# MarioPasc/MGA-YOLO

Hardware: AMD Instinct MI355X
Metric: images/s (MaskCBAM fwd+bwd step at P3/P4/P5, YOLOv8n 640x640) (higher is better)
Workload: dtype f32; 1 GPU; YOLOv8n+MGA-CBAM P3/P4/P5, 32x640x640 synthetic per GPU, fp32 (BASELINE.json configs[1]); batch_per_gpu=32, global_batch=32, parallelism=dp1, launch=hipGraph replay, 1 graph/step, handoff_kernels=True

## Files before the change

mga_yolo_amd/csrc/api_bwd.hip:

```cpp
#include "host.cuh"
#include "bwd.cuh"
#include "nhwc_bwd.cuh"

static int backward_args(const mgacbam_bwd_level_t& L, NhwcBwdArgs& N, Sig& sig) {
  const bool nhwc = (L.flags & MGACBAM_LAYOUT_NHWC) != 0;
  if (!L.x || !L.gy || !L.ctx || !L.scratch || !L.gx) return fail(MGACBAM_E_NULL, "backward: x / gy / ctx / scratch / gx is NULL");
  if (!L.gw1 || !L.gb1 || !L.gw2 || !L.gb2 || !L.gwsa || !L.gbeta) return fail(MGACBAM_E_NULL, "backward: NULL parameter-gradient pointer");
  if (L.gmask && !L.mask) return fail(MGACBAM_E_NULL, "backward: gmask requested but mask is NULL");
  if (int e = check_level("backward", L)) return e;
  const int VEC = level_vec(nhwc, L.C, L.H, L.W, L.dtype);
  const size_t need = VEC * elem_size(L.dtype);
  if (!aligned_to(L.x, need) || !aligned_to(L.gy, need) || !aligned_to(L.gx, need) || !aligned_to(L.ctx, 16) ||
      !aligned_to(L.scratch, 16) || (L.gmask && !aligned_to(L.gmask, nhwc ? 4 : 16)) || (nhwc && L.mask && !aligned_to(L.mask, 4)))
    return fail(MGACBAM_E_ALIGN, "backward%s: x/gy/gx must be %zu-byte aligned, ctx/scratch 16-byte", nhwc ? " (NHWC)" : "", need);
  const ScratchLayout SL = scratch_layout(L.B, L.C, L.H, L.W, L.p.hidden, L.p.k, nhwc, VEC);
  if (int e = check_ctx_capacity("backward", L)) return e;
  if (int e = check_capacity("backward", "scratch", SL.total, L.scratch_bytes)) return e;
  BwdArgs& A = N.a;
  A.x = L.x; A.mask = L.mask; A.gy = L.gy; A.gx = L.gx; A.gmask = L.gmask;
  A.gw1 = L.gw1; A.gb1 = L.gb1; A.gw2 = L.gw2; A.gb2 = L.gb2; A.gwsa = L.gwsa; A.gbeta = L.gbeta;
  level_setup(L, A);
  A.s = scratch_ptrs(L.scratch, SL);
  A.nconv = A.g.B * conv_tiles(A.t, A.g.H, A.g.W);
  A.nwsa = A.g.B * wsa_tiles(A.t, A.g.H, A.g.W);
  A.npg = params_blocks(A.g);
  A.merged = 0;
  A.make_proj = 0;
  A.vec = VEC;
  sig = Sig{L.dtype, VEC, L.mask != nullptr, L.p.k, L.gmask != nullptr, 0};
  if (nhwc) {
    N.n = nhwc_geo(L.C, L.H, L.W, VEC);
    N.ncb = (L.C + kNhwcFoldC - 1) / kNhwcFoldC;
    A.nt = N.n.nchunk;
    A.ncg = N.ncb;
    A.bflag0 = A.cflag0 = A.mbflag0 = A.mcflag0 = A.wflag0 = A.sflag0 = 0;
    sig.nhwc = 1;
    sig.weight = L.C;
    return 0;
  }
  A.nt = chan_tiles(A.t, A.g.H, A.g.W, VEC);
  A.ncg = 0;
  const SyncLayout S = sync_layout(L.B, L.C, static_cast<size_t>(L.H) * L.W);
  A.bflag0 = static_cast<int>(S.bflag); A.cflag0 = static_cast<int>(S.cflag);
  A.mbflag0 = static_cast<int>(S.mbflag); A.mcflag0 = static_cast<int>(S.mcflag);
  A.wflag0 = static_cast<int>(S.wflag); A.sflag0 = static_cast<int>(S.sflag);
  sig.weight = L.C * A.t.chan_tx;
  const bool have = (L.flags & MGACBAM_BWD_HAVE_PROJ) != 0;
  const bool make = !have && L.dtype == MGACBAM_F32 && reduce1_smem(A.g, VEC, true) <= 64 * 1024;
  sig.proj = L.gmask != nullptr;
  A.g.proj_h = (L.gmask && L.p.hidden <= MGACBAM_PROJ_MAX_HIDDEN && (have || make)) ? L.p.hidden : 0;
  A.make_proj = A.g.proj_h > 0 && make;
  return 0;
}

static size_t reduce2_smem(const Tune& t) { return (64 + static_cast<size_t>(std::max(kPghLds, kBlock / t.pool_tx))) * sizeof(float); }
static int launch_convT(Group<BwdArgs>& G, int k, hipStream_t st) {
  auto kernel = with_k(k, [](auto kk) { return k_bwd_convT<kk.value>; });
  return launch_group("k_bwd_convT", kernel, G, [](const BwdArgs& a) { return a.nconv; }, [&](const BwdArgs& a) { return convT_smem(a.t, k); }, st);
}
static int launch_wsa(Group<BwdArgs>& G, int k, hipStream_t st) {
  auto kernel = with_k(k, [](auto kk) { return k_bwd_wsa<kk.value>; });
  return launch_group("k_bwd_wsa", kernel, G, [](const BwdArgs& a) { return a.nwsa; }, [&](const BwdArgs& a) { return wsa_smem(a.t, k); }, st);
}
static int launch_params(Group<BwdArgs>& G, hipStream_t st) {
  return launch_group("k_bwd_params", k_bwd_params, G, [](const BwdArgs& a) { return a.npg; }, [](const BwdArgs& a) { return params_smem(a.g); }, st);
}

static int backward_group(BwdArgs* lv, int n, const Sig& sig, int stages, hipStream_t st) {
  constexpr int kReduce2MaxCpt = 4;
  const int cpt = group_cpt(lv, n, kReduce2MaxCpt);
  for (int l = 0; l < n; ++l) {
    lv[l].t.pool_cpt = cpt;
    const int cpb = (kBlock / lv[l].t.pool_tx) * cpt;
    lv[l].ncg = (lv[l].g.C + cpb - 1) / cpb;
  }
  Group<BwdArgs> G = make_group(lv, n);

  bool fold = (stages & MGACBAM_BWD_FOLD) && (stages & MGACBAM_BWD_REDUCE1) && (stages & MGACBAM_BWD_CONVT);
  for (int l = 0; l < n && fold; ++l) {
    const int TP = lv[l].t.chan_tx * sig.vec;
    fold = TP >= kSyncPx && TP >= lv[l].g.W && 8 * (((lv[l].t.conv_th + lv[l].g.k) * lv[l].g.W + TP - 1) / TP + 1) <= 512 &&
           lv[l].nconv <= lv[l].g.B * lv[l].nflag;
  }
  bool mkproj = false;
// ... 23 lines not shown
      return with_bool(mkproj, [&](auto pj) { return k_bwd_r12<elem_t<decltype(t)>, v.value, c.value, pj.value>; }); }); });
    if (int e = launch("k_bwd_r12", kernel, tot, kBlock, smem, st, R)) return e;
    for (int l = 0; l < n; ++l) G.lv[l] = lv[l];
  }
  if (fold && !merge) {
    auto kernel = with_elem_vec(sig.dtype, sig.vec, [&](auto t, auto v) { return with_k7(sig.k, [&](auto k) {
      return with_bool(mkproj, [&](auto pj) { return k_bwd_reduce1_fold<elem_t<decltype(t)>, v.value, k.value, pj.value>; }); }); });
    if (int e = launch_group("k_bwd_reduce1_fold", kernel, G, [](const BwdArgs& a) { return xcd_grid(a.g.B, a.nt) + pad8(a.nconv); },
                             [&](const BwdArgs& a) { return std::max(reduce1_smem(a.g, sig.vec, a.make_proj), convT_smem(a.t, sig.k)); },
                             st)) return e;
  }
  if ((stages & MGACBAM_BWD_REDUCE1) && !fold) {
    auto kernel = with_elem_vec(sig.dtype, sig.vec, [&](auto t, auto v) {
      return with_bool(mkproj, [&](auto pj) { return k_bwd_reduce1<elem_t<decltype(t)>, v.value, pj.value>; }); });
    if (int e = launch_group("k_bwd_reduce1", kernel, G, [](const BwdArgs& a) { return xcd_grid(a.g.B, a.nt); },
                             [&](const BwdArgs& a) { return reduce1_smem(a.g, sig.vec, a.make_proj); }, st)) return e;
  }
  if ((stages & MGACBAM_BWD_CONVT) && !fold)
    if (int e = launch_convT(G, sig.k, st)) return e;
  const bool fuse_pg = fuse && (stages & MGACBAM_BWD_APPLY) && (stages & MGACBAM_BWD_PARAMGRAD);
  const bool fuse_wsa = fuse && (stages & MGACBAM_BWD_REDUCE2) && (stages & MGACBAM_BWD_WSA) && sig.k == 7;
  if ((stages & MGACBAM_BWD_REDUCE2) && !merge) {
    auto kernel = with_elem_vec(sig.dtype, sig.vec, [&](auto t, auto v) { return with_cpt(cpt, [&](auto c) {
      return with_bool(fuse_wsa, [&](auto fw) { return k_bwd_reduce2<elem_t<decltype(t)>, v.value, c.value, fw.value>; }); }); });
    if (int e = launch_group("k_bwd_reduce2", kernel, G,
                             [&](const BwdArgs& a) { return (fuse_wsa ? pad8(a.nwsa) : 0) + sweep_blocks(a, a.t.pool_tx, cpt); },
                             [&](const BwdArgs& a) { return std::max(reduce2_smem(a.t), fuse_wsa ? wsa_smem(a.t, sig.k) : 0); }, st)) return e;
  }
  if ((stages & MGACBAM_BWD_WSA) && !fuse_wsa && !merge)
    if (int e = launch_wsa(G, sig.k, st)) return e;
  if ((stages & MGACBAM_BWD_PARAMGRAD) && !fuse_pg)
    if (int e = launch_params(G, st)) return e;
  if (stages & MGACBAM_BWD_APPLY) {
    auto kernel = with_elem_vec(sig.dtype, sig.vec, [&](auto t, auto v) { return with_bool(sig.gmask, [&](auto gm) {
      return with_bool(fuse_pg, [&](auto pg) { return k_bwd_apply<elem_t<decltype(t)>, v.value, gm.value, pg.value>; }); }); });
    if (int e = launch_group("k_bwd_apply", kernel, G, [&](const BwdArgs& a) { return (fuse_pg ? pad8(a.npg) : 0) + xcd_grid(a.g.B, a.nt); },
                             [&](const BwdArgs& a) { return std::max(bwd_apply_smem(a.g, sig.vec), fuse_pg ? params_smem(a.g) : 0); }, st)) return e;
  }
  return 0;
}

static int backward_group_nhwc(NhwcBwdArgs* lv, int n, const Sig& sig, int stages, hipStream_t st) {
  Group<NhwcBwdArgs> G = make_group(lv, n);
  Group<BwdArgs> GB;
  GB.n = n;
  for (int l = 0; l < n; ++l) GB.lv[l] = lv[l].a;
  auto chunks = [](const NhwcBwdArgs& a) { return xcd_grid(a.a.g.B, a.n.nchunk); };
  if (stages & MGACBAM_BWD_REDUCE1) {
    auto kernel = with_elem_vec8(sig.dtype, sig.vec, [](auto t, auto v) { return k_bwd_reduce1_nhwc<elem_t<decltype(t)>, v.value>; });
    if (int e = launch_group("k_bwd_reduce1_nhwc", kernel, G, chunks,
                             [&](const NhwcBwdArgs& a) { return nhwc_reduce1_smem(a.a.g, sig.vec); }, st)) return e;
  }
  if (stages & MGACBAM_BWD_CONVT)
    if (int e = launch_convT(GB, sig.k, st)) return e;
  if (stages & MGACBAM_BWD_REDUCE2) {
    auto kernel = with_elem_vec8(sig.dtype, sig.vec, [](auto t, auto v) { return k_bwd_reduce2_nhwc<elem_t<decltype(t)>, v.value>; });
    if (int e = launch_group("k_bwd_reduce2_nhwc", kernel, G, chunks, [](const NhwcBwdArgs& a) { return nhwc_reduce2_smem(a.a.g); }, st)) return e;
    if (int e = launch_group("k_bwd_fold_nhwc", k_bwd_fold_nhwc, G, [](const NhwcBwdArgs& a) { return a.a.g.B * a.ncb; }, 0, st)) return e;
  }
  if (stages & MGACBAM_BWD_WSA)
    if (int e = launch_wsa(GB, sig.k, st)) return e;
  if (stages & MGACBAM_BWD_PARAMGRAD)
    if (int e = launch_params(GB, st)) return e;
  if (stages & MGACBAM_BWD_APPLY) {
    auto kernel = with_elem_vec8(sig.dtype, sig.vec, [&](auto t, auto v) {
      return with_bool(sig.gmask, [&](auto gm) { return k_bwd_apply_nhwc<elem_t<decltype(t)>, v.value, gm.value>; }); });
    if (int e = launch_group("k_bwd_apply_nhwc", kernel, G, [](const NhwcBwdArgs& a) { return xcd_grid(a.a.g.B, a.n.ntile); },
                             [](const NhwcBwdArgs& a) { return nhwc_bwd_apply_smem(a.a.g); }, st)) return e;
// ... 14 lines not shown
```

mga_yolo_amd/csrc/args.cuh:

```cuda
#pragma once
#include <stddef.h>
#include <stdint.h>

namespace mgacbam {

struct Geo {
  int B, C, H, W, HW;
  int hidden, k;
  int use_sigmoid;
  float thr, eps;
  int proj_h;
};
constexpr int kProjMax = 4;
constexpr int kGateR = 16;
constexpr int kSyncPx = 16;

struct CtxPtrs {
  float* S; float* use; float* den;
  float* avg; float* mx; float* mavg;
  int* valid; int* amax;
  float* h_avg; float* h_mx; float* ca;
  float* planes; int* cidx; float* sa;
  float* proj;
  int* sync;
};

struct ParamPtrs { const float* w1; const float* b1; const float* w2; const float* b2; const float* wsa; const float* beta; };

struct Tune {
  int pool_tx;
  int pool_cpt;
  int chan_tx;
  int conv_twq;
  int conv_th;
  int wsa_th;
  int apply_rows;
  int gate_rows;
  int gate_tx;
  int gate_span;
};

struct FwdArgs {
  const void* x; const float* mask; void* y;
  CtxPtrs c; ParamPtrs p; Geo g; Tune t;
  int nflag;
  int fused;
  unsigned spin_limit;
  int fault;
  long long* trace;
};

struct ScratchPtrs {
  float* A_part;
  float* gpre;
  float* gplanes;
  float* gwsa_part;
  float* gz;
  float* gbq;
  float* gh_avg;
  float* gh_mx;
  float* pgh;
};

struct BwdArgs {
  const void* x; const float* mask; const void* gy; void* gx; float* gmask;
  float* gw1; float* gb1; float* gw2; float* gb2; float* gwsa; float* gbeta;
  CtxPtrs c; ParamPtrs p; ScratchPtrs s; Geo g; Tune t;
  int nt;
  int nconv;
  int nwsa;
  int npg;
  int ncg;
  int nflag;
  int bflag0;
  int cflag0;
  int wflag0;
  int sflag0;
  int mbflag0, mcflag0;
  int make_proj;
  int merged;
  unsigned spin_limit;
  int vec;
  long long* trace;
};

struct NhwcGeo {
  int cs, lcs;
  int ng;
  int ch;
  int ntile;
  int rp;
  int nchunk;
};
constexpr int kNhwcMaxChunks = 64;
// ... 14 lines not shown
```

mga_yolo_amd/csrc/bwd.cuh:

```cuda
#pragma once
#include "args.cuh"
#include "common.cuh"
#include "tile.cuh"

namespace mgacbam {

constexpr int kPghLds = 2048;

template <typename T, int VEC, bool FOLD = false, bool PROJ = false>
__device__ __forceinline__ void bwd_reduce1_body(const BwdArgs& A, const int bid, float* smem) {
  constexpr int HP = kProjMax;
  static_assert(HP % 4 == 0, "the W1 rows of a channel are read as float4");
  const Geo& g = A.g;
  const int tid = threadIdx.x;
  const int TX = A.t.chan_tx, lt = ilog2(TX);
  const int tx = tid & (TX - 1), ty = tid >> lt, TY = kBlock >> lt;
  const int nv = g.HW / VEC;
  const int ntile = A.nt;
  int b, tile;
  if (!xcd_sample_part(bid, g.B, ntile, b, tile)) return;
  const int i = tile * TX + tx;
  const bool active = i < nv;
  const int ii = active ? i : nv - 1;
  const size_t base = static_cast<size_t>(b) * g.C * g.HW + static_cast<size_t>(ii) * VEC;
  const T* xp = static_cast<const T*>(A.x) + base;
  const T* gp = static_cast<const T*>(A.gy) + base;
  const float a = softplusf_(*A.p.beta);
  float* s_ca = smem;
  float* s_aq = smem + g.C;
  const bool proj = PROJ && A.make_proj;
  float* s_w1t = smem + ((3 * g.C + 3) & ~3);
  float* sm = proj ? s_w1t + g.C * HP : s_aq + 2 * g.C;
  for (int c = tid; c < g.C; c += kBlock) s_ca[c] = A.c.ca[static_cast<size_t>(b) * g.C + c];
  if (PROJ) {
    if (proj) {
      for (int idx = tid; idx < g.C * HP; idx += kBlock) {
        const int c = idx / HP, j = idx - c * HP;
        s_w1t[idx] = j < g.proj_h ? A.p.w1[static_cast<size_t>(j) * g.C + c] : 0.f;
      }
    }
  }

  float sav[VEC];
  load_vec<float, VEC>(A.c.sa + static_cast<size_t>(b) * g.HW + static_cast<size_t>(ii) * VEC, sav);
  const float live = active ? 1.f : 0.f;
  float accp[VEC];
#pragma unroll
  for (int e = 0; e < VEC; ++e) accp[e] = 0.f;
  float accP[PROJ ? HP : 1][VEC];
#pragma unroll
  for (int j = 0; j < (PROJ ? HP : 1); ++j)
#pragma unroll
    for (int e = 0; e < VEC; ++e) accP[j][e] = 0.f;
  __syncthreads();

#pragma unroll 4
  for (int c = ty; c < g.C; c += TY) {
    float xv[VEC], gv[VEC];
    load_vec<T, VEC>(xp + static_cast<size_t>(c) * g.HW, xv);
    load_vec<T, VEC>(gp + static_cast<size_t>(c) * g.HW, gv);
    const float cac = s_ca[c];
    if (PROJ) {
      if (proj) {
        float w[HP];
#pragma unroll
        for (int q4 = 0; q4 < HP / 4; ++q4) {
          const float4 wv = *reinterpret_cast<const float4*>(s_w1t + c * HP + 4 * q4);
          w[4 * q4] = wv.x; w[4 * q4 + 1] = wv.y; w[4 * q4 + 2] = wv.z; w[4 * q4 + 3] = wv.w;
        }
#pragma unroll
        for (int j = 0; j < HP; ++j)
#pragma unroll
          for (int e = 0; e < VEC; ++e) accP[j][e] += w[j] * xv[e];
      }
    }
    float pa = 0.f, pq = 0.f;
#pragma unroll
    for (int e = 0; e < VEC; ++e) {
      const float p = xv[e] * gv[e] * live;
      accp[e] += cac * p;
      pa += p * sav[e];
      pq += p * (cac * sav[e] - 1.f);
    }
    pa = wave_group_sum(pa, TX);
    pq = wave_group_sum(pq, TX);
    if (tx == 0) { s_aq[c] = pa; s_aq[g.C + c] = pq; }
  }
#pragma unroll
  for (int e = 0; e < VEC; ++e) sm[tid * VEC + e] = accp[e];
  __syncthreads();
// ... 16 lines not shown
    } else {
      store_vec<float, VEC>(gq, gpre);
    }
  }
  if (FOLD) handoff_publish(A.c.sync + A.bflag0 + static_cast<size_t>(b) * A.nflag + tile);
  if (PROJ) {
    if (proj) {
#pragma unroll
      for (int half = 0; half < HP / 4; ++half) {
        if (half * 4 >= g.proj_h) break;
        if (!FOLD || half) __syncthreads();
#pragma unroll
        for (int jj = 0; jj < 4; ++jj)
#pragma unroll
          for (int e = 0; e < VEC; ++e) sm[(jj * kBlock + tid) * VEC + e] = accP[half * 4 + jj][e];
        __syncthreads();
        if (ty == 0 && active) {
#pragma unroll
          for (int jj = 0; jj < 4; ++jj) {
            const int j = half * 4 + jj;
            if (j < g.proj_h) {
              float pv[VEC];
#pragma unroll
              for (int e = 0; e < VEC; ++e) pv[e] = accP[j][e];
              for (int r = 1; r < TY; ++r)
#pragma unroll
                for (int e = 0; e < VEC; ++e) pv[e] += sm[(jj * kBlock + r * TX + tx) * VEC + e];
              store_vec<float, VEC>(A.c.proj + (static_cast<size_t>(b) * g.proj_h + j) * g.HW + static_cast<size_t>(i) * VEC, pv);
            }
          }
        }
      }
    }
  }
}

template <typename T, int VEC, bool PROJ>
__global__ __launch_bounds__(kBlock) void k_bwd_reduce1(const Group<BwdArgs> G) {
  extern __shared__ __align__(16) float smem[];
  int local;
  const int l = find_level(G, blockIdx.x, local);
  bwd_reduce1_body<T, VEC, false, PROJ>(G.lv[l], local, smem);
}

template <int K, bool COH>
__device__ __forceinline__ void bwd_convT_body(const BwdArgs& A, const int local, float* smem) {
  const Geo& g = A.g;
  const int k = K ? K : g.k;
  const ConvTile c = conv_tile(g, A.t, k, local, A.t.conv_th);
  const int tid = threadIdx.x;
  float* wts = smem;
  float* tg = smem + ((3 * k * k + 3) & ~3);
  for (int i = tid; i < 3 * k * k; i += kBlock) wts[i] = A.p.wsa[i];
  const float* gpre = A.s.gpre + static_cast<size_t>(c.b) * g.HW;
  bool bad = false;
  if (COH) {
    int* own = A.c.sync + A.cflag0 + local;
    const int gen = static_cast<int>(static_cast<unsigned>(ld_agent(own)) + 1u);
    const int TP = A.t.chan_tx * A.vec;
    const int ra = max(c.y0 - c.pad, 0), rb = min(c.y0 + c.TH - 1 + c.pad, g.H - 1);
    bad = handoff_wait(A.c.sync + A.bflag0 + static_cast<size_t>(c.b) * A.nflag, (ra * g.W) / TP, ((rb + 1) * g.W - 1) / TP, gen,
                       A.c.sync + static_cast<size_t>(g.B) * A.nflag, A.spin_limit);
    if (tid == 0 && !A.merged) __hip_atomic_fetch_add(own, 1, __ATOMIC_RELAXED, __HIP_MEMORY_SCOPE_AGENT);
  }
  stage_window<8>(tg, 1, c.PH, c.PW, c.y0 - c.pad, c.x0 - c.pad, g, [&](int, int off) { return COH ? ld_agent(gpre + off) : gpre[off]; });
  __syncthreads();
  const int TWQ = A.t.conv_twq;
  const int py = tid / TWQ, q = tid - py * TWQ;
  constexpr int KK = K ? K : 1;
  const bool publish = COH && A.merged;
  if (py >= c.TH && !publish) return;
// ... 31 lines not shown
#pragma unroll
          for (int e = 0; e < 4; ++e) acc[p][e] += wv * row[e + j];
        }
      }
    }
  }
  const int yg = c.y0 + py;
  if (py < c.TH && yg < g.H) {
#pragma unroll
    for (int e = 0; e < 4; ++e) {
      const int xg = c.x0 + q * 4 + e;
      if (xg < g.W) {
#pragma unroll
        for (int p = 0; p < 3; ++p) {
          float* dst = A.s.gplanes + (static_cast<size_t>(c.b) * 3 + p) * g.HW + yg * g.W + xg;
          const float v = bad ? __builtin_nanf("") : acc[p][e];
          if (publish) st_agent(dst, v); else *dst = v;
        }
      }
    }
  }
  if (publish) handoff_publish(A.c.sync + A.cflag0 + local);
}

template <int K>
__global__ __launch_bounds__(kBlock) void k_bwd_convT(const Group<BwdArgs> G) {
  extern __shared__ __align__(16) float smem[];
  int local;
  const int lvl = find_level(G, blockIdx.x, local);
  bwd_convT_body<K, false>(G.lv[lvl], local, smem);
}

template <typename T, int VEC, int K, bool PROJ>
__global__ __launch_bounds__(kBlock) void k_bwd_reduce1_fold(const Group<BwdArgs> G) {
  extern __shared__ __align__(16) float smem[];
  int local;
  const int l = find_level(G, blockIdx.x, local);
  const BwdArgs& A = G.lv[l];
  const int tiles = ((A.g.B + 7) / 8) * 8 * A.nt;
  if (local >= tiles) {
    if (local - tiles < A.nconv) bwd_convT_body<K, true>(A, local - tiles, smem);
    return;
  }
  bwd_reduce1_body<T, VEC, true, PROJ>(A, local, smem);
}

template <int K, bool COH = false>
__device__ __forceinline__ void bwd_wsa_body(const BwdArgs& A, const int local, float* smem) {
  const Geo& g = A.g;
  const int k = K ? K : g.k;
  const ConvTile c = conv_tile(g, A.t, k, local, A.t.wsa_th);
  const int tid = threadIdx.x;
  const int plane_elems = c.PH * c.PW;
  float* tg = smem;
  float* tp = tg + plane_elems;
  float* accs = tp + 3 * plane_elems;
  const float* gpre = A.s.gpre + static_cast<size_t>(c.b) * g.HW;
  const float* pl = A.c.planes + static_cast<size_t>(c.b) * 3 * g.HW;
  bool bad = false;
  if (COH) {
    int* own = A.c.sync + A.wflag0 + local;
    const int gen = static_cast<int>(static_cast<unsigned>(ld_agent(own)) + 1u);
    const int TP = A.t.chan_tx * A.vec;
    const int ra = max(c.y0 - c.pad, 0), rb = min(c.y0 + c.TH - 1 + c.pad, g.H - 1);
    bad = handoff_wait(A.c.sync + A.bflag0 + static_cast<size_t>(c.b) * A.nflag, (ra * g.W) / TP, ((rb + 1) * g.W - 1) / TP, gen,
                       A.c.sync + static_cast<size_t>(g.B) * A.nflag, A.spin_limit);
    if (tid == 0) __hip_atomic_fetch_add(own, 1, __ATOMIC_RELAXED, __HIP_MEMORY_SCOPE_AGENT);
// ... 31 lines not shown
      for (int j = 0; j < KK; ++j) accs[item * KK + j] = acc[j];
    }
    __syncthreads();
    for (int o = tid; o < nout; o += kBlock) {
      const int pi = o / KK, j = o - pi * KK;
      float sum = 0.f;
      for (int r = 0; r < c.TH; ++r) sum += accs[(pi * c.TH + r) * KK + j];
      if (COH && bad) sum = __builtin_nanf("");
      A.s.gwsa_part[static_cast<size_t>(o) * A.nwsa + local] = sum;
    }
  } else {
    for (int o = tid; o < nout; o += kBlock) {
      const int p = o / (k * k), r = o - p * k * k;
      const int i = r / k, j = r - i * k;
      const float* pp = tp + p * plane_elems + i * c.PW + j;
      const float* gg = tg + c.pad * c.PW + c.pad;
      float sum = 0.f;
      for (int yy = 0; yy < c.TH; ++yy)
        for (int xx = 0; xx < c.TW; ++xx) sum += gg[yy * c.PW + xx] * pp[yy * c.PW + xx];
      A.s.gwsa_part[static_cast<size_t>(o) * A.nwsa + local] = sum;
    }
  }
}

template <int K>
__global__ __launch_bounds__(kBlock) void k_bwd_wsa(const Group<BwdArgs> G) {
  extern __shared__ __align__(16) float smem[];
  int local;
  const int lvl = find_level(G, blockIdx.x, local);
  bwd_wsa_body<K>(G.lv[lvl], local, smem);
}

typedef unsigned int v4u32_t __attribute__((ext_vector_type(4)));
typedef float v4f32_t __attribute__((ext_vector_type(4)));
template <int VEC>
__device__ __forceinline__ void load_plane_agent(__amdgpu_buffer_rsrc_t rsrc, const int elem, float (&out)[VEC]) {
  if constexpr (VEC % 4 == 0) {
#pragma unroll
    for (int q = 0; q < VEC / 4; ++q) {
      const v4u32_t v = __builtin_amdgcn_raw_buffer_load_b128(rsrc, (elem + 4 * q) * 4, 0, 16);
      const v4f32_t f = __builtin_bit_cast(v4f32_t, v);
      out[4 * q] = f.x; out[4 * q + 1] = f.y; out[4 * q + 2] = f.z; out[4 * q + 3] = f.w;
    }
  } else {
#pragma unroll
    for (int e = 0; e < VEC; ++e) out[e] = __builtin_bit_cast(float, __builtin_amdgcn_raw_buffer_load_b32(rsrc, (elem + e) * 4, 0, 16));
  }
}

template <typename T, int VEC, int CPT, bool COH = false>
__device__ __forceinline__ void bwd_reduce2_body(const BwdArgs& A, const int bid, float* red) {
  const Geo& g = A.g;
  const int tid = threadIdx.x;
  const int TX = A.t.pool_tx, lt = ilog2(TX);
  const int tx = tid & (TX - 1), ty = tid >> lt, TY = kBlock >> lt;
  const int CPB = TY * CPT;
  const int ncg = (g.C + CPB - 1) / CPB;
  int b, cg;
  if (!xcd_sample_part(bid, g.B, ncg, b, cg)) return;
  const int c0 = cg * CPB + ty * CPT;
  const int nv = g.HW / VEC;
  const float invC = 1.f / static_cast<float>(g.C);

  const T* xr[CPT];
  int cj[CPT];
#pragma unroll
  for (int j = 0; j < CPT; ++j) {
// ... 108 lines not shown
  extern __shared__ __align__(16) float smem[];
  int local;
  const int l = find_level(G, blockIdx.x, local);
  const BwdArgs& A = G.lv[l];
  if (ROLES) {
    const int npad = (A.nwsa + 7) & ~7;
    if (local < npad) {
      if (local < A.nwsa) {
        TRACE_MARK(A.trace, blockIdx.x, 0);
        bwd_wsa_body<7>(A, local, smem);
#ifdef MGACBAM_TRACE
        asm volatile("s_waitcnt vmcnt(0)" ::: "memory");
        __syncthreads();
        TRACE_MARK(A.trace, blockIdx.x, 5);
#endif
      }
      return;
    }
    local -= npad;
  }
  TRACE_MARK(A.trace, blockIdx.x, 0);
  bwd_reduce2_body<T, VEC, CPT>(A, local, smem);
#ifdef MGACBAM_TRACE
  asm volatile("s_waitcnt vmcnt(0)" ::: "memory");
  TRACE_MARK(A.trace, blockIdx.x, 10);
#endif
}

struct R12Group {
  Group<BwdArgs> g;
  int seg[4][kGroupMax + 1];
};
template <typename T, int VEC, int CPT, bool PROJ>
__global__ __launch_bounds__(kBlock) void k_bwd_r12(const R12Group R) {
  extern __shared__ __align__(16) float smem[];
  const int bid = blockIdx.x;
  int p = 0;
#pragma unroll
  for (int q = 1; q < 4; ++q)
    if (bid >= R.seg[q][0]) p = q;
  int l = 0;
#pragma unroll
  for (int i = 1; i < kGroupMax; ++i)
    if (i < R.g.n && bid >= R.seg[p][i]) l = i;
  const int local = bid - R.seg[p][l];
  const BwdArgs& A = R.g.lv[l];
#ifdef MGACBAM_TRACE
  TRACE_MARK(A.trace, blockIdx.x, 0);
  if (A.trace && threadIdx.x == 0) A.trace[static_cast<size_t>(blockIdx.x) * 16 + 14] = p + 1;
#endif
  if (p == 0) bwd_reduce1_body<T, VEC, true, PROJ>(A, local, smem);
  else if (p == 1) { if (local < A.nconv) bwd_convT_body<7, true>(A, local, smem); }
  else if (p == 2) { if (local < A.nwsa) bwd_wsa_body<7, true>(A, local, smem); }
  else bwd_reduce2_body<T, VEC, CPT, true>(A, local, smem);
#ifdef MGACBAM_TRACE
  asm volatile("s_waitcnt vmcnt(0)" ::: "memory");
  __syncthreads();
  TRACE_MARK(A.trace, blockIdx.x, 10);
#endif
}

__device__ __forceinline__ void bwd_params_body(const BwdArgs& A, const int local, float* sm, float* red) {
  const Geo& g = A.g;
  const int C = g.C, h = g.hidden, B = g.B, kk3 = 3 * g.k * g.k;
  const int nb2 = (C + kBlock - 1) / kBlock, nb_wsa = (kk3 + 3) / 4;
  const int tid = threadIdx.x, wave = tid >> 6, lane = tid & 63;
  if (local < h) {
// ... 57 lines not shown
#pragma unroll 8
    for (int b = 0; b < B; ++b) acc += A.s.gz[static_cast<size_t>(b) * C + c];
    A.gb2[c] = 2.f * acc;
    return;
  }
  if (local < h + nb2 + nb_wsa) {
    const int o = (local - h - nb2) * 4 + wave;
    if (o >= kk3) return;
    const float* part = A.s.gwsa_part + static_cast<size_t>(o) * A.nwsa;
    float acc = 0.f;
#pragma unroll 4
    for (int t = lane; t < A.nwsa; t += kWave) acc += part[t];
    acc = wave_group_sum(acc, kWave);
    if (lane == 0) A.gwsa[o] = acc;
    return;
  }
  {
    float acc = 0.f;
#pragma unroll 8
    for (int o = tid; o < B * C; o += kBlock) acc += A.s.gbq[o];
    acc = block_sum(acc, tid, red);
    if (tid == 0) *A.gbeta = sigmoidf_(*A.p.beta) * acc;
  }
}

__global__ __launch_bounds__(kBlock) void k_bwd_params(const Group<BwdArgs> G) {
  extern __shared__ __align__(16) float sm[];
  __shared__ float red[8];
  int local;
  const int lvl = find_level(G, blockIdx.x, local);
  bwd_params_body(G.lv[lvl], local, sm, red);
}

template <typename T, int VEC, bool GMASK>
__device__ __forceinline__ void bwd_apply_body(const BwdArgs& A, const int bid, float* smem, float* red) {
  constexpr int UN = 2;
  const Geo& g = A.g;
  const int tid = threadIdx.x;
  const int TX = A.t.chan_tx, lt = ilog2(TX);
  const int tx = tid & (TX - 1), ty = tid >> lt, TY = kBlock >> lt;
  const int nv = g.HW / VEC;
  const int ntile = (nv + TX - 1) / TX;
  int b, tile;
  if (!xcd_sample_part(bid, g.B, ntile, b, tile)) return;
  const int i = tile * TX + tx;
  const bool active = i < nv;
  const int ii = active ? i : nv - 1;
  const size_t base = static_cast<size_t>(b) * g.C * g.HW + static_cast<size_t>(ii) * VEC;
  const T* xp = static_cast<const T*>(A.x) + base;
  const T* gp = static_cast<const T*>(A.gy) + base;
  T* op = static_cast<T*>(A.gx) + base;
  const float a = softplusf_(*A.p.beta);
  const float N = static_cast<float>(g.HW);
  const bool has_mask = A.mask != nullptr;
  const size_t po = static_cast<size_t>(b) * g.HW + static_cast<size_t>(ii) * VEC;

  const int gid = blockIdx.x;
  TRACE_HWID(A.trace, gid);
  TRACE_MARK(A.trace, gid, 0);
  float sav[VEC], g0[VEC], g1[VEC], sv[VEC], wA[VEC];
  int ci[VEC];
  load_vec<float, VEC>(A.c.sa + po, sav);
  load_vec<float, VEC>(A.s.gplanes + static_cast<size_t>(b) * 3 * g.HW + static_cast<size_t>(ii) * VEC, g0);
  load_vec<float, VEC>(A.s.gplanes + (static_cast<size_t>(b) * 3 + 1) * g.HW + static_cast<size_t>(ii) * VEC, g1);
  load_vec<float, VEC>(A.c.planes + (static_cast<size_t>(b) * 3 + 2) * g.HW + static_cast<size_t>(ii) * VEC, sv);
  load_ivec<VEC>(A.c.cidx + po, ci);
  const float use = A.c.use[b], den = A.c.den[b];
  const float invC = 1.f / static_cast<float>(g.C);
#pragma unroll
  for (int e = 0; e < VEC; ++e) {
    g1[e] *= invC;
    sav[e] *= a;
    wA[e] = has_mask ? (use * sv[e] / den + (1.f - use) / N) : 1.f / N;
  }
  const int* amax = A.c.amax + static_cast<size_t>(b) * g.C;
  float accp[VEC];
#pragma unroll
  for (int e = 0; e < VEC; ++e) accp[e] = 0.f;

  const bool need_x = GMASK && g.proj_h == 0;
  float g0v[UN][VEC], x0v[UN][VEC];
#pragma unroll
  for (int u = 0; u < UN; ++u) {
    const size_t co = static_cast<size_t>(min(ty + u * TY, g.C - 1)) * g.HW;
    load_vec<T, VEC>(gp + co, g0v[u]);
    if (GMASK) { if (need_x) load_vec<T, VEC>(xp + co, x0v[u]); }
  }

  float4* s_q = reinterpret_cast<float4*>(smem);
  int* s_am = reinterpret_cast<int*>(smem + 4 * g.C);
  float* s_gh = smem + 5 * g.C;
  float* sm = s_gh + 2 * g.hidden;
  const int h = g.hidden;
  const float live = (has_mask && A.c.S[b] >= g.eps) ? 1.f : 0.f;
  float kpart = 0.f;
  constexpr int kEarlyH = 8;
  const bool early = g.C <= kBlock && h <= kEarlyH;
  float rw1[kEarlyH], rca = 0.f, rmavg = 0.f;
  int rvalid = 0, ramax = 0;
  if (early) {
    const int c = min(tid, g.C - 1);
    const size_t o = static_cast<size_t>(b) * g.C + c;
    rca = A.c.ca[o]; rmavg = A.c.mavg[o]; rvalid = A.c.valid[o]; ramax = amax[c];
#pragma unroll
    for (int j = 0; j < kEarlyH; ++j) rw1[j] = A.p.w1[static_cast<size_t>(min(j, h - 1)) * g.C + c];
  }
  {
    const float* pg = A.s.pgh + static_cast<size_t>(b) * A.ncg * h;
    const int hh = h < kBlock ? h : kBlock;
    const int G_ = kBlock / hh;
    const int j0 = tid % hh, k0 = tid / hh;
    for (int jb = 0; jb < h; jb += hh) {
      const int j = jb + j0;
      float p = 0.f;
      if (k0 < G_ && j < h)
        for (int cg = k0; cg < A.ncg; cg += G_) p += pg[cg * h + j];
      sm[tid] = p;
      __syncthreads();
      if (k0 == 0 && j < h) {
// ... 46 lines not shown
  auto emit = [&](const float (&gv)[VEC], const float (&xv)[VEC], int c) {
    float ov[VEC];
    const float4 q = s_q[c];
    const int am = s_am[c] - ii * VEC;
#pragma unroll
    for (int e = 0; e < VEC; ++e) {
      float r = gv[e] * ((1.f - a) + sav[e] * q.x);
      r += q.x * ((ci[e] == c ? g0[e] : 0.f) + g1[e]);
      r += q.y * wA[e] + q.w;
      r += (am == e) ? q.z : 0.f;
      ov[e] = r;
      if (GMASK) { if (need_x) accp[e] += q.y * xv[e]; }
    }
    if (active) store_vec<T, VEC>(op + static_cast<size_t>(c) * g.HW, ov);
  };
#pragma unroll
  for (int u = 0; u < UN; ++u) {
    const int c = ty + u * TY;
    if (c < g.C) emit(g0v[u], x0v[u], c);
  }
#pragma unroll 4
  for (int c = ty + UN * TY; c < g.C; c += TY) {
    float gv[VEC], xv[VEC];
    load_vec<T, VEC>(gp + static_cast<size_t>(c) * g.HW, gv);
    if (GMASK) { if (need_x) load_vec<T, VEC>(xp + static_cast<size_t>(c) * g.HW, xv); }
    emit(gv, xv, c);
  }
  TRACE_MARK(A.trace, gid, 3);
  if (GMASK) {
    if (need_x) {
#pragma unroll
      for (int e = 0; e < VEC; ++e) sm[tid * VEC + e] = accp[e];
      __syncthreads();
    }
    if (ty == 0 && active) {
      if (need_x) {
        for (int r = 1; r < TY; ++r) {
          const int o = (r * TX + tx) * VEC;
#pragma unroll
          for (int e = 0; e < VEC; ++e) accp[e] += sm[o + e];
        }
      } else {
        for (int j = 0; j < g.proj_h; ++j) {
          float pv[VEC];
          load_vec<float, VEC>(A.c.proj + (static_cast<size_t>(b) * g.proj_h + j) * g.HW + static_cast<size_t>(i) * VEC, pv);
          const float gh = s_gh[j];
#pragma unroll
          for (int e = 0; e < VEC; ++e) accp[e] += gh * pv[e];
        }
      }
      float g2[VEC], gm[VEC];
      load_vec<float, VEC>(A.s.gplanes + (static_cast<size_t>(b) * 3 + 2) * g.HW + static_cast<size_t>(i) * VEC, g2);
#pragma unroll
      for (int e = 0; e < VEC; ++e) {
        const float gs = g2[e] + (use / den) * (accp[e] - kb);
        gm[e] = g.use_sigmoid ? gs * sv[e] * (1.f - sv[e]) : gs;
      }
      store_vec<float, VEC>(A.gmask + static_cast<size_t>(b) * g.HW + static_cast<size_t>(i) * VEC, gm);
    }
  }
#ifdef MGACBAM_TRACE
  asm volatile("s_waitcnt vmcnt(0)" ::: "memory");
  __syncthreads();
  TRACE_MARK(A.trace, gid, 10);
#endif
}

template <typename T, int VEC, bool GMASK, bool ROLES>
__global__ __launch_bounds__(kBlock) void k_bwd_apply(const Group<BwdArgs> G) {
  extern __shared__ __align__(16) float smem[];
  __shared__ float red[8];
  int local;
  const int l = find_level(G, blockIdx.x, local);
  const BwdArgs& A = G.lv[l];
  if (ROLES) {
    const int npad = (A.npg + 7) & ~7;
    if (local < npad) {
      if (local < A.npg) {
        TRACE_MARK(A.trace, blockIdx.x, 0);
        bwd_params_body(A, local, smem, red);
#ifdef MGACBAM_TRACE
        asm volatile("s_waitcnt vmcnt(0)" ::: "memory");
        __syncthreads();
        TRACE_MARK(A.trace, blockIdx.x, 9);
#endif
      }
      return;
    }
    local -= npad;
  }
  bwd_apply_body<T, VEC, GMASK>(A, local, smem, red);
}

}
```

mga_yolo_amd/csrc/host.cuh:

```cuda
#pragma once
#include "../../include/mgacbam.h"

#include <hip/hip_runtime.h>
#include <stdarg.h>
#include <stdio.h>
#include <stdlib.h>
#include <string.h>

#include <algorithm>
#include <atomic>
#include <map>
#include <mutex>
#include <type_traits>
#include <utility>

#include "args.cuh"
#include "common.cuh"

using namespace mgacbam;

inline thread_local char g_err[512] = "";
static int fail(int code, const char* fmt, ...) {
  va_list ap;
  va_start(ap, fmt);
// ... 203 lines not shown

static int conv_tiles(const Tune& t, int H, int W) {
  const int TW = t.conv_twq * 4;
  return ((W + TW - 1) / TW) * ((H + t.conv_th - 1) / t.conv_th);
}
static int wsa_tiles(const Tune& t, int H, int W) {
  const int TW = t.conv_twq * 4;
  return ((W + TW - 1) / TW) * ((H + t.wsa_th - 1) / t.wsa_th);
}
static int chan_tiles(const Tune& t, int H, int W, int vec) {
  const int nv = H * W / vec;
  return (nv + t.chan_tx - 1) / t.chan_tx;
}

static int nhwc_vec(int C, int dtype) { return (dtype != MGACBAM_F32 && C % 8 == 0) ? 8 : (C % 4 == 0 ? 4 : 1); }
static int level_vec(bool nhwc, int C, int H, int W, int dtype) { return nhwc ? nhwc_vec(C, dtype) : vec_of(H, W); }
static NhwcGeo nhwc_geo(int C, int H, int W, int vec) {
  NhwcGeo n;
  n.ng = (C + vec - 1) / vec;
  n.cs = std::max(4, std::min(pow2_ceil(n.ng), 64));
  n.lcs = 0;
  while ((1 << n.lcs) < n.cs) ++n.lcs;
  n.ch = (kBlock / n.cs) * (vec == 8 ? 4 : 8);
  n.ntile = static_cast<int>((static_cast<long long>(H) * W + n.ch - 1) / n.ch);
  n.rp = (n.ntile + kNhwcMaxChunks - 1) / kNhwcMaxChunks;
  n.nchunk = (n.ntile + n.rp - 1) / n.rp;
  return n;
}
static int nhwc_fold_blocks(const Geo& g) { return g.B * ((g.C + kNhwcFoldC - 1) / kNhwcFoldC); }
static size_t nhwc_ws_bytes(int B, int C, int H, int W, int vec) {
  return static_cast<size_t>(B) * nhwc_geo(C, H, W, vec).nchunk * (4 * static_cast<size_t>(C) + 4) * sizeof(float);
}

struct ScratchLayout { size_t A_part, gpre, gplanes, gwsa_part, gz, gbq, gh_avg, gh_mx, pgh, total; };
static ScratchLayout scratch_layout(int B, int C, int H, int W, int hidden, int k, bool nhwc, int vec) {
  const Tune t = choose_tune(B, C, H, W, k);
  const size_t HW = static_cast<size_t>(H) * W, BC = static_cast<size_t>(B) * C;
  const size_t nwsa = static_cast<size_t>(B) * wsa_tiles(t, H, W);
  ScratchLayout L;
  Carver cv;
  L.A_part = cv.take(nhwc ? 3 * BC * nhwc_geo(C, H, W, vec).nchunk : 2 * BC * chan_tiles(t, H, W, vec));
  L.gpre = cv.take(B * HW); L.gplanes = cv.take(static_cast<size_t>(B) * 3 * HW);
  L.gwsa_part = cv.take(nwsa * 3 * k * k);
  L.gz = cv.take(BC); L.gbq = cv.take(BC);
  L.gh_avg = cv.take(static_cast<size_t>(B) * hidden); L.gh_mx = cv.take(static_cast<size_t>(B) * hidden);
  const size_t cpg = nhwc ? kNhwcFoldC : kBlock / t.pool_tx;
  L.pgh = cv.take(static_cast<size_t>(B) * ((C + cpg - 1) / cpg) * hidden);
  L.total = cv.total;
  return L;
}
static ScratchPtrs scratch_ptrs(void* p, const ScratchLayout& L) {
  return ScratchPtrs{at(p, L.A_part), at(p, L.gpre), at(p, L.gplanes), at(p, L.gwsa_part), at(p, L.gz), at(p, L.gbq),
                     at(p, L.gh_avg), at(p, L.gh_mx), at(p, L.pgh)};
}
static size_t ws_bytes_any(int B, int C, int H, int W, bool nhwc) {
  if (!nhwc) return 0;
  return std::max(nhwc_ws_bytes(B, C, H, W, nhwc_vec(C, MGACBAM_F32)), nhwc_ws_bytes(B, C, H, W, nhwc_vec(C, MGACBAM_F16)));
}
static size_t scratch_bytes_any(int B, int C, int H, int W, int hidden, int k, bool nhwc) {
  return std::max(scratch_layout(B, C, H, W, hidden, k, nhwc, level_vec(nhwc, C, H, W, MGACBAM_F32)).total,
                  scratch_layout(B, C, H, W, hidden, k, nhwc, level_vec(nhwc, C, H, W, MGACBAM_F16)).total);
}

static int check_capacity(const char* what, const char* buf, size_t want, size_t got) {
  if (got < want)
    return fail(MGACBAM_E_SIZE, "%s: %s holds %zu bytes, this shape needs %zu under the current knobs (query the size again after "
                "mgacbam_reload_env(); a size cached across a knob change or taken for another shape is stale)", what, buf, got, want);
  return 0;
}

static size_t elem_size(int dtype) { return dtype == MGACBAM_F32 ? 4 : 2; }
static bool aligned_to(const void* p, size_t a) { return (reinterpret_cast<uintptr_t>(p) % a) == 0; }

static int check_dtype(const char* what, int dtype) {
  if (dtype < MGACBAM_F32 || dtype > MGACBAM_BF16) return fail(MGACBAM_E_DTYPE, "%s: dtype %d", what, dtype);
  return 0;
}

template <typename T> struct Ty { using type = T; };
template <int V> using Int = std::integral_constant<int, V>;
template <typename F>
static auto with_elem(int dtype, F f) {
  if (dtype == MGACBAM_F32) return f(Ty<float>{});
  if (dtype == MGACBAM_F16) return f(Ty<__half>{});
  return f(Ty<bf16_t>{});
}
// ... 89 lines not shown
}
static int xcd_grid(int B, int parts) { return ((B + 7) / 8) * 8 * parts; }
static int pad8(int n) { return (n + 7) & ~7; }
template <typename Args>
static int sweep_blocks(const Args& a, int tx, int cpt) {
  const int cpb = (kBlock / tx) * cpt;
  return xcd_grid(a.g.B, (a.g.C + cpb - 1) / cpb);
}
static size_t convT_smem(const Tune& t, int k) {
  return (((3 * k * k + 3) & ~3) + static_cast<size_t>(t.conv_th + k - 1) * (t.conv_twq * 4 + k - 1)) * sizeof(float);
}
static size_t wsa_smem(const Tune& t, int k) {
  return (4 * static_cast<size_t>(t.wsa_th + k - 1) * (t.conv_twq * 4 + k - 1) + static_cast<size_t>(3 * k * t.wsa_th) * k) * sizeof(float);
}
static size_t params_smem(const Geo& g) { return (3 * static_cast<size_t>(g.B) + 2 * kBlock) * sizeof(float); }
static int params_blocks(const Geo& g) { return g.hidden + (g.C + kBlock - 1) / kBlock + (3 * g.k * g.k + 3) / 4 + 1; }
static size_t chan_smem(const Geo& g, int vec, bool proj) {
  return (3 * static_cast<size_t>(g.C) + 2 * g.hidden + (proj ? static_cast<size_t>(g.C) * kProjMax : 0) + 4 * kBlock * vec) * sizeof(float);
}
static size_t apply_smem(const Geo& g, const Tune& t, int vec) {
  return (((3 * g.k * g.k + 3) & ~3) + 3 * static_cast<size_t>(t.apply_rows) * (g.W + g.k - 1) + t.chan_tx * vec + g.C) * sizeof(float);
}
static size_t gate_smem(const Geo& g, const Tune& t, int vec) {
  const size_t head = (g.C + 3) & ~3;
  const size_t role = 3 * static_cast<size_t>(g.C) + 2 * g.hidden;
  const size_t conv = ((3 * g.k * g.k + 3) & ~3) + 3 * static_cast<size_t>(t.gate_rows) * (g.W + g.k - 1) + static_cast<size_t>(t.gate_tx) * vec;
  return std::max(role, head + std::max(conv, static_cast<size_t>(3) * kBlock * vec)) * sizeof(float);
}
static int gate_tiles(const Tune& t, int H, int W, int vec) {
  const int nv = H * W / vec;
  return (nv + t.gate_tx - 1) / t.gate_tx;
}
static size_t bwd_apply_smem(const Geo& g, int vec) { return (5 * static_cast<size_t>(g.C) + 2 * g.hidden + kBlock * vec) * sizeof(float); }
static size_t reduce1_smem(const Geo& g, int vec, bool proj) {
  if (!proj) return (3 * static_cast<size_t>(g.C) + kBlock * vec) * sizeof(float);
  return (((3 * static_cast<size_t>(g.C) + 3) & ~static_cast<size_t>(3)) + static_cast<size_t>(g.C) * kProjMax + 4 * kBlock * vec) * sizeof(float);
}
static size_t mlp_smem(const Geo& g) { return (3 * static_cast<size_t>(g.C) + 2 * g.hidden) * sizeof(float); }
static size_t nhwc_pool_smem(const Geo& g) { return 4 * static_cast<size_t>(g.C) * sizeof(float); }
static size_t nhwc_chan_smem(const Geo& g) { return static_cast<size_t>(g.C) * sizeof(float); }
static size_t nhwc_apply_smem(const Geo& g, const Tune& t, const NhwcGeo& n) {
  return (((3 * g.k * g.k + 3) & ~3) + 3 * static_cast<size_t>(t.apply_rows) * (g.W + g.k - 1) + n.ch + g.C) * sizeof(float);
}
static size_t nhwc_reduce1_smem(const Geo& g, int vec) {
  return (3 * ((static_cast<size_t>(g.C) + 3) & ~static_cast<size_t>(3)) + 2 * kBlock * vec) * sizeof(float);
}
static size_t nhwc_reduce2_smem(const Geo& g) { return static_cast<size_t>(g.C) * sizeof(float); }
static size_t nhwc_bwd_apply_smem(const Geo& g) { return (5 * static_cast<size_t>(g.C) + 2 * g.hidden) * sizeof(float); }

template <typename Args, typename Fn>
static int fill_starts(Group<Args>& G, const Args* lv, int n, Fn blocks_of) {
  int tot = 0;
  for (int l = 0; l < n; ++l) { G.start[l] = tot; tot += blocks_of(lv[l]); }
  G.start[n] = tot;
  return tot;
}
template <typename Args>
static Group<Args> make_group(const Args* lv, int n) {
  Group<Args> G;
  G.n = n;
  for (int l = 0; l < n; ++l) G.lv[l] = lv[l];
  return G;
}
template <typename Args, typename SmemOf>
static size_t group_smem(const Group<Args>& G, SmemOf smem_of) {
  if constexpr (std::is_convertible_v<SmemOf, size_t>) {
    return smem_of;
  } else {
// ... 53 lines not shown
```

Before: 166,200 images/s.

## Compute wide hidden-projection in reduce1 via MFMA and skip x reload in apply

For f32 NCHW levels whose hidden size is between 4 and 16, reduce1 now computes the W1·x projection per pixel with 16x16x4 f32 MFMA instructions and stores it to a new scratch buffer. The backward apply kernel then reads these precomputed projection rows instead of reloading x over all channels to build the gmask gradient. This trades a full x re-read for an extra B*hidden*HW scratch write and read, adds cross-wave LDS reduction in reduce1, and sets waves_per_eu hints on the PROJ kernels.

Result: faster. 170,300 images/s (median of 6 runs) (+2.4%).

```diff
diff --git a/mga_yolo_amd/csrc/api_bwd.hip b/mga_yolo_amd/csrc/api_bwd.hip
--- a/mga_yolo_amd/csrc/api_bwd.hip
+++ b/mga_yolo_amd/csrc/api_bwd.hip
@@ -50,6 +50,11 @@
   sig.proj = L.gmask != nullptr;
   A.g.proj_h = (L.gmask && L.p.hidden <= MGACBAM_PROJ_MAX_HIDDEN && (have || make)) ? L.p.hidden : 0;
   A.make_proj = A.g.proj_h > 0 && make;
+  if (L.gmask && L.dtype == MGACBAM_F32 && wide_proj_shape(L.B, L.C, L.H, L.W, L.p.hidden, false, VEC, A.t)) {
+    A.g.proj_h = L.p.hidden;
+    A.make_proj = 2;
+    A.c.proj = A.s.proj;
+  }
   return 0;
 }
 
@@ -139,8 +144,16 @@
   if ((stages & MGACBAM_BWD_PARAMGRAD) && !fuse_pg)
     if (int e = launch_params(G, st)) return e;
   if (stages & MGACBAM_BWD_APPLY) {
+    bool nox = sig.gmask && sig.dtype == MGACBAM_F32 && sig.vec == 4;
+    for (int l = 0; l < n; ++l) nox = nox && lv[l].g.proj_h > 0;
     auto kernel = with_elem_vec(sig.dtype, sig.vec, [&](auto t, auto v) { return with_bool(sig.gmask, [&](auto gm) {
-      return with_bool(fuse_pg, [&](auto pg) { return k_bwd_apply<elem_t<decltype(t)>, v.value, gm.value, pg.value>; }); }); });
+      return with_bool(fuse_pg, [&](auto pg) {
+        using T = elem_t<decltype(t)>;
+        if constexpr (std::is_same_v<T, float> && v.value == 4 && gm.value) {
+          return nox ? k_bwd_apply<T, v.value, gm.value, pg.value, false> : k_bwd_apply<T, v.value, gm.value, pg.value, true>;
+        } else {
+          return k_bwd_apply<T, v.value, gm.value, pg.value, true>;
+        } }); }); });
     if (int e = launch_group("k_bwd_apply", kernel, G, [&](const BwdArgs& a) { return (fuse_pg ? pad8(a.npg) : 0) + xcd_grid(a.g.B, a.nt); },
                              [&](const BwdArgs& a) { return std::max(bwd_apply_smem(a.g, sig.vec), fuse_pg ? params_smem(a.g) : 0); }, st)) return e;
   }
diff --git a/mga_yolo_amd/csrc/args.cuh b/mga_yolo_amd/csrc/args.cuh
--- a/mga_yolo_amd/csrc/args.cuh
+++ b/mga_yolo_amd/csrc/args.cuh
@@ -12,6 +12,7 @@
   int proj_h;
 };
 constexpr int kProjMax = 4;
+constexpr int kProjWide = 16;
 constexpr int kGateR = 16;
 constexpr int kSyncPx = 16;
 
@@ -60,6 +61,7 @@
   float* gh_avg;
   float* gh_mx;
   float* pgh;
+  float* proj;
 };
 
 struct BwdArgs {
diff --git a/mga_yolo_amd/csrc/bwd.cuh b/mga_yolo_amd/csrc/bwd.cuh
--- a/mga_yolo_amd/csrc/bwd.cuh
+++ b/mga_yolo_amd/csrc/bwd.cuh
@@ -6,6 +6,7 @@
 namespace mgacbam {
 
 constexpr int kPghLds = 2048;
+typedef float v4f32_t __attribute__((ext_vector_type(4)));
 
 template <typename T, int VEC, bool FOLD = false, bool PROJ = false>
 __device__ __forceinline__ void bwd_reduce1_body(const BwdArgs& A, const int bid, float* smem) {
@@ -28,9 +29,10 @@
   const float a = softplusf_(*A.p.beta);
   float* s_ca = smem;
   float* s_aq = smem + g.C;
-  const bool proj = PROJ && A.make_proj;
+  const bool proj = PROJ && A.make_proj == 1;
+  const bool wide = PROJ && A.make_proj == 2;
   float* s_w1t = smem + ((3 * g.C + 3) & ~3);
-  float* sm = proj ? s_w1t + g.C * HP : s_aq + 2 * g.C;
+  float* sm = proj ? s_w1t + g.C * HP : wide ? s_w1t : s_aq + 2 * g.C;
   for (int c = tid; c < g.C; c += kBlock) s_ca[c] = A.c.ca[static_cast<size_t>(b) * g.C + c];
   if (PROJ) {
     if (proj) {
@@ -54,8 +56,44 @@
     for (int e = 0; e < VEC; ++e) accP[j][e] = 0.f;
   __syncthreads();
 
+  bool mfma_done = false;
+  if constexpr (PROJ && VEC == 4 && sizeof(T) == 4) {
+    if (wide) {
+      static_assert(HP == 4, "accP is the four accumulator quads of the MFMA form");
+      v4f32_t m[4];
+#pragma unroll
+      for (int e = 0; e < 4; ++e) m[e] = v4f32_t{accP[0][e], accP[1][e], accP[2][e], accP[3][e]};
+      const bool arow = tx < g.proj_h;
+      const float* w1r = A.p.w1 + static_cast<size_t>(arow ? tx : 0) * g.C;
 #pragma unroll 4
-  for (int c = ty; c < g.C; c += TY) {
+      for (int c0 = 0; c0 < g.C; c0 += TY) {
+        const bool ok = c0 + ty < g.C;
+        const int c = ok ? c0 + ty : g.C - 1;
+        float xv[VEC], gv[VEC];
+        load_vec<T, VEC>(xp + static_cast<size_t>(c) * g.HW, xv);
+        load_vec<T, VEC>(gp + static_cast<size_t>(c) * g.HW, gv);
+        const float aw = (arow && ok) ? w1r[c] : 0.f;
+        const float cac = s_ca[c];
+        float pa = 0.f, pq = 0.f;
+#pragma unroll
+        for (int e = 0; e < VEC; ++e) {
+          m[e] = __builtin_amdgcn_mfma_f32_16x16x4f32(aw, ok ? xv[e] : 0.f, m[e], 0, 0, 0);
+          const float p = ok ? xv[e] * gv[e] * live : 0.f;
+          accp[e] += cac * p;
+          pa += p * sav[e];
+          pq += p * (cac * sav[e] - 1.f);
+        }
+        pa = wave_group_sum(pa, TX);
+        pq = wave_group_sum(pq, TX);
+        if (tx == 0 && ok) { s_aq[c] = pa; s_aq[g.C + c] = pq; }
+      }
+#pragma unroll
+      for (int e = 0; e < 4; ++e) { accP[0][e] = m[e].x; accP[1][e] = m[e].y; accP[2][e] = m[e].z; accP[3][e] = m[e].w; }
+      mfma_done = true;
+    }
+  }
+#pragma unroll 4
+  for (int c = mfma_done ? g.C : ty; c < g.C; c += TY) {
     float xv[VEC], gv[VEC];
     load_vec<T, VEC>(xp + static_cast<size_t>(c) * g.HW, xv);
     load_vec<T, VEC>(gp + static_cast<size_t>(c) * g.HW, gv);
@@ -138,11 +176,38 @@
         }
       }
     }
+    if constexpr (VEC == 4 && sizeof(T) == 4) {
+      if (wide) {
+        const int wave = tid >> 6, lane = tid & (kWave - 1);
+        if (!FOLD) __syncthreads();
+        if (wave) {
+#pragma unroll
+          for (int r = 0; r < 4; ++r)
+#pragma unroll
+            for (int e = 0; e < 4; ++e) sm[(((wave - 1) * 4 + r) * 4 + e) * kWave + lane] = accP[r][e];
+        }
+        __syncthreads();
+        if (wave == 0) {
+          for (int w = 0; w < kBlock / kWave - 1; ++w)
+#pragma unroll
+            for (int r = 0; r < 4; ++r)
+#pragma unroll
+              for (int e = 0; e < 4; ++e) accP[r][e] += sm[((w * 4 + r) * 4 + e) * kWave + lane];
+          if (active) {
+#pragma unroll
+            for (int r = 0; r < 4; ++r) {
+              const int j = 4 * ty + r;
+              if (j < g.proj_h) store_vec<float, VEC>(A.c.proj + (static_cast<size_t>(b) * g.proj_h + j) * g.HW + static_cast<size_t>(i) * VEC, accP[r]);
+            }
+          }
+        }
+      }
+    }
   }
 }
 
 template <typename T, int VEC, bool PROJ>
-__global__ __launch_bounds__(kBlock) void k_bwd_reduce1(const Group<BwdArgs> G) {
+__global__ __launch_bounds__(kBlock) __attribute__((amdgpu_waves_per_eu(PROJ ? 2 : 1))) void k_bwd_reduce1(const Group<BwdArgs> G) {
   extern __shared__ __align__(16) float smem[];
   int local;
   const int l = find_level(G, blockIdx.x, local);
@@ -240,7 +305,7 @@
 }
 
 template <typename T, int VEC, int K, bool PROJ>
-__global__ __launch_bounds__(kBlock) void k_bwd_reduce1_fold(const Group<BwdArgs> G) {
+__global__ __launch_bounds__(kBlock) __attribute__((amdgpu_waves_per_eu(PROJ ? 2 : 1))) void k_bwd_reduce1_fold(const Group<BwdArgs> G) {
   extern __shared__ __align__(16) float smem[];
   int local;
   const int l = find_level(G, blockIdx.x, local);
@@ -338,7 +403,6 @@
 }
 
 typedef unsigned int v4u32_t __attribute__((ext_vector_type(4)));
-typedef float v4f32_t __attribute__((ext_vector_type(4)));
 template <int VEC>
 __device__ __forceinline__ void load_plane_agent(__amdgpu_buffer_rsrc_t rsrc, const int elem, float (&out)[VEC]) {
   if constexpr (VEC % 4 == 0) {
@@ -513,7 +577,7 @@
   int seg[4][kGroupMax + 1];
 };
 template <typename T, int VEC, int CPT, bool PROJ>
-__global__ __launch_bounds__(kBlock) void k_bwd_r12(const R12Group R) {
+__global__ __launch_bounds__(kBlock) __attribute__((amdgpu_waves_per_eu(PROJ ? 2 : 1))) void k_bwd_r12(const R12Group R) {
   extern __shared__ __align__(16) float smem[];
   const int bid = blockIdx.x;
   int p = 0;
@@ -637,7 +701,7 @@
   bwd_params_body(G.lv[lvl], local, sm, red);
 }
 
-template <typename T, int VEC, bool GMASK>
+template <typename T, int VEC, bool GMASK, bool NEEDX>
 __device__ __forceinline__ void bwd_apply_body(const BwdArgs& A, const int bid, float* smem, float* red) {
   constexpr int UN = 2;
   const Geo& g = A.g;
@@ -683,13 +747,18 @@
 #pragma unroll
   for (int e = 0; e < VEC; ++e) accp[e] = 0.f;
 
-  const bool need_x = GMASK && g.proj_h == 0;
+  const bool need_x = NEEDX && GMASK && g.proj_h == 0;
   float g0v[UN][VEC], x0v[UN][VEC];
 #pragma unroll
   for (int u = 0; u < UN; ++u) {
     const size_t co = static_cast<size_t>(min(ty + u * TY, g.C - 1)) * g.HW;
     load_vec<T, VEC>(gp + co, g0v[u]);
     if (GMASK) { if (need_x) load_vec<T, VEC>(xp + co, x0v[u]); }
+  }
+  const bool prow = GMASK && sizeof(T) == 4 && g.proj_h > 0 && g.proj_h <= TY;
+  float pjv[VEC];
+  if (GMASK) {
+    if (prow && ty < g.proj_h) load_vec<float, VEC>(A.c.proj + (static_cast<size_t>(b) * g.proj_h + ty) * g.HW + static_cast<size_t>(ii) * VEC, pjv);
   }
 
   float4* s_q = reinterpret_cast<float4*>(smem);
@@ -802,6 +871,12 @@
 #pragma unroll
       for (int e = 0; e < VEC; ++e) sm[tid * VEC + e] = accp[e];
       __syncthreads();
+    } else if (prow) {
+      if (ty < g.proj_h) {
+#pragma unroll
+        for (int e = 0; e < VEC; ++e) sm[tid * VEC + e] = pjv[e];
+      }
+      __syncthreads();
     }
     if (ty == 0 && active) {
       if (need_x) {
@@ -809,6 +884,13 @@
           const int o = (r * TX + tx) * VEC;
 #pragma unroll
           for (int e = 0; e < VEC; ++e) accp[e] += sm[o + e];
+        }
+      } else if (prow) {
+        for (int j = 0; j < g.proj_h; ++j) {
+          const float gh = s_gh[j];
+          const int o = (j * TX + tx) * VEC;
+#pragma unroll
+          for (int e = 0; e < VEC; ++e) accp[e] += gh * sm[o + e];
         }
       } else {
         for (int j = 0; j < g.proj_h; ++j) {
@@ -836,7 +918,7 @@
 #endif
 }
 
-template <typename T, int VEC, bool GMASK, bool ROLES>
+template <typename T, int VEC, bool GMASK, bool ROLES, bool NEEDX = true>
 __global__ __launch_bounds__(kBlock) void k_bwd_apply(const Group<BwdArgs> G) {
   extern __shared__ __align__(16) float smem[];
   __shared__ float red[8];
@@ -859,7 +941,7 @@
     }
     local -= npad;
   }
-  bwd_apply_body<T, VEC, GMASK>(A, local, smem, red);
-}
-
-}
+  bwd_apply_body<T, VEC, GMASK, NEEDX>(A, local, smem, red);
+}
+
+}
diff --git a/mga_yolo_amd/csrc/host.cuh b/mga_yolo_amd/csrc/host.cuh
--- a/mga_yolo_amd/csrc/host.cuh
+++ b/mga_yolo_amd/csrc/host.cuh
@@ -259,7 +259,11 @@
   return static_cast<size_t>(B) * nhwc_geo(C, H, W, vec).nchunk * (4 * static_cast<size_t>(C) + 4) * sizeof(float);
 }
 
-struct ScratchLayout { size_t A_part, gpre, gplanes, gwsa_part, gz, gbq, gh_avg, gh_mx, pgh, total; };
+struct ScratchLayout { size_t A_part, gpre, gplanes, gwsa_part, gz, gbq, gh_avg, gh_mx, pgh, proj, total; };
+static bool wide_proj_shape(int B, int C, int H, int W, int hidden, bool nhwc, int vec, const Tune& t) {
+  return !nhwc && hidden > kProjMax && hidden <= kProjWide && vec == 4 && t.chan_tx == 16 &&
+         static_cast<size_t>(B) * C * H * W * sizeof(float) >= (size_t(1) << 20);
+}
 static ScratchLayout scratch_layout(int B, int C, int H, int W, int hidden, int k, bool nhwc, int vec) {
   const Tune t = choose_tune(B, C, H, W, k);
   const size_t HW = static_cast<size_t>(H) * W, BC = static_cast<size_t>(B) * C;
@@ -273,12 +277,13 @@
   L.gh_avg = cv.take(static_cast<size_t>(B) * hidden); L.gh_mx = cv.take(static_cast<size_t>(B) * hidden);
   const size_t cpg = nhwc ? kNhwcFoldC : kBlock / t.pool_tx;
   L.pgh = cv.take(static_cast<size_t>(B) * ((C + cpg - 1) / cpg) * hidden);
+  L.proj = cv.take(wide_proj_shape(B, C, H, W, hidden, nhwc, vec, t) ? static_cast<size_t>(B) * hidden * HW : 0);
   L.total = cv.total;
   return L;
 }
 static ScratchPtrs scratch_ptrs(void* p, const ScratchLayout& L) {
   return ScratchPtrs{at(p, L.A_part), at(p, L.gpre), at(p, L.gplanes), at(p, L.gwsa_part), at(p, L.gz), at(p, L.gbq),
-                     at(p, L.gh_avg), at(p, L.gh_mx), at(p, L.pgh)};
+                     at(p, L.gh_avg), at(p, L.gh_mx), at(p, L.pgh), at(p, L.proj)};
 }
 static size_t ws_bytes_any(int B, int C, int H, int W, bool nhwc) {
   if (!nhwc) return 0;
@@ -434,8 +439,9 @@
   return (nv + t.gate_tx - 1) / t.gate_tx;
 }
 static size_t bwd_apply_smem(const Geo& g, int vec) { return (5 * static_cast<size_t>(g.C) + 2 * g.hidden + kBlock * vec) * sizeof(float); }
-static size_t reduce1_smem(const Geo& g, int vec, bool proj) {
+static size_t reduce1_smem(const Geo& g, int vec, int proj) {
   if (!proj) return (3 * static_cast<size_t>(g.C) + kBlock * vec) * sizeof(float);
+  if (proj == 2) return (((3 * static_cast<size_t>(g.C) + 3) & ~static_cast<size_t>(3)) + 3 * 16 * kWave) * sizeof(float);
   return (((3 * static_cast<size_t>(g.C) + 3) & ~static_cast<size_t>(3)) + static_cast<size_t>(g.C) * kProjMax + 4 * kBlock * vec) * sizeof(float);
 }
 static size_t mlp_smem(const Geo& g) { return (3 * static_cast<size_t>(g.C) + 2 * g.hidden) * sizeof(float); }
```
